# TGoldC/Motion-Planning-for-Autonomous-Driving-with-MPC

Hardware: AMD Instinct MI355X
Metric: MPC steps/sec (N=30, nx=6 nu=2) at batch=4096 (higher is better)
Workload: dtype f64; 1 GPU; N=30 nx=6 nu=2 bicycle lane-following, batch=4096/GPU, tol 1e-8; mode=converged, gpu=AMD Radeon Graphics

## Files before the change

motion-planning-for-autonomous-driving-with-mpc_amd/csrc/mpc_solve_plan.h:

```cpp
#pragma once
#include <algorithm>
#include <cctype>
#include <cstdlib>
#include <cstring>
#include <string>

#include "mpc_host_common.h"

namespace mpc {

struct Knobs {
    int pipeline, hybrid, hybrid_bx, hybrid_live, pipe_help, pipe_test_abort, pipe_xcd_mask, pipe_early;
    int rescue, rescue_wg, rescue_alone, loop_async, sync_spin, max_batch, friction_lb, bound_mask, big_wg, groups, poison;
    int timing;
    Knobs();
};
enum class KnobParse {
    ON,
    INT,
    FLAG,
    MASK,
    FRIC,
};
struct KnobDef { const char* name; int Knobs::*field; int dflt; KnobParse parse; };
inline constexpr KnobDef KNOBS[] = {
    {"pipeline", &Knobs::pipeline, 1, KnobParse::ON},           {"hybrid", &Knobs::hybrid, 1, KnobParse::INT},
    {"hybrid_bx", &Knobs::hybrid_bx, 0, KnobParse::INT},        {"hybrid_live", &Knobs::hybrid_live, -1, KnobParse::INT},
    {"pipe_help", &Knobs::pipe_help, -1, KnobParse::INT},       {"pipe_test_abort", &Knobs::pipe_test_abort, 0, KnobParse::FLAG},
    {"pipe_xcd_mask", &Knobs::pipe_xcd_mask, 0, KnobParse::MASK}, {"rescue", &Knobs::rescue, 1, KnobParse::ON},
    {"rescue_wg", &Knobs::rescue_wg, 1, KnobParse::INT},        {"rescue_alone", &Knobs::rescue_alone, 0, KnobParse::FLAG},
    {"loop_async", &Knobs::loop_async, 1, KnobParse::ON},       {"sync_spin", &Knobs::sync_spin, 1, KnobParse::ON},
    {"max_batch", &Knobs::max_batch, 0, KnobParse::INT},        {"friction_lb", &Knobs::friction_lb, 0, KnobParse::FRIC},
    {"bound_mask", &Knobs::bound_mask, 1, KnobParse::INT},      {"big_wg", &Knobs::big_wg, 0, KnobParse::FLAG},
    {"groups", &Knobs::groups, 0, KnobParse::INT},              {"poison", &Knobs::poison, 0, KnobParse::FLAG},
    {"timing", &Knobs::timing, 0, KnobParse::INT},               {"pipe_early", &Knobs::pipe_early, -1, KnobParse::INT},
};
inline Knobs::Knobs() { for (const KnobDef& e : KNOBS) this->*e.field = e.dflt; }
inline const KnobDef* find_knob(const char* name) {
    for (const KnobDef& e : KNOBS) if (name && strcmp(name, e.name) == 0) return &e;
    return nullptr;
}
inline int set_knob(Knobs& k, const char* name, const char* value) {
    const KnobDef* e = find_knob(name);
    if (!e) return MPC_ERR_INVALID;
    int v = e->dflt;
    if (value) {
        const long iv = strtol(value, nullptr, 0);
        switch (e->parse) {
            case KnobParse::ON: v = value[0] != '0'; break;
            case KnobParse::INT: v = (int)iv; break;
            case KnobParse::FLAG: v = (value[0] == '\0' ? 1 : (int)iv) != 0; break;
            case KnobParse::MASK: v = (int)(uint32_t)strtoul(value, nullptr, 0); break;
            case KnobParse::FRIC: v = strcmp(value, "ipopt") == 0 ? 1 : strcmp(value, "nlp") == 0 ? 0 : (int)iv; break;
        }
    }
    k.*e->field = v;
    return MPC_OK;
}
inline int get_knob(const Knobs& k, const char* name, long* out) {
    const KnobDef* e = find_knob(name);
    if (!e) return MPC_ERR_INVALID;
    *out = e->parse == KnobParse::MASK ? (long)(uint32_t)(k.*e->field) : (long)(k.*e->field);
    return MPC_OK;
}
inline void knobs_from_env(Knobs& k) {
    for (const KnobDef& e : KNOBS) {
        std::string env = "MPCGPU_";
        for (const char* c = e.name; *c; ++c) env += (char)toupper(*c);
        const char* v = getenv(env.c_str());
        if (v) (void)set_knob(k, e.name, v);
    }
}

constexpr int TIMING_STAGE = 1,
              TIMING_PIPE = 2,
              TIMING_WG = 4,
              TIMING_START = 8,
              TIMING_WG_TRACE = 16;

constexpr int STAGE_MAX_THREADS = 512;
constexpr int MAX_GROUPS = 4;
constexpr int MAX_POLL_IT = 1024;
constexpr size_t LDS_MAX = 160 * 1024 - 1024;

#ifndef MPC_STAGE_STASH
#define MPC_STAGE_STASH 1
#endif
template <int NX> struct Stash {
    static constexpr int rows(bool has_ou) { return 4 * (NX + 2) + 2 * 3 + (has_ou ? 2 * 3 : 0) + 3 + 2 * NX; }
};

constexpr uint32_t REF_BOUND_VM = 0x33u;
constexpr uint32_t REF_DENSE_LO = 0x31u, REF_DENSE_HI = 0x33u;

constexpr int RIC_DEPTH = 4;
constexpr int RIC_DEPTH_F = 10;

constexpr uint32_t PIPE_X_STRIDE = 64;
enum PipeXcdWord : uint32_t { PX_ARRIVE = 0, PX_HEAD = 16, PX_TAIL = 32, PX_FINISHED = 48, PX_HO_TICKET = 56 };
constexpr uint32_t PIPE_ABORT = 8 * PIPE_X_STRIDE;
constexpr uint32_t HO_BUCKETS = 4;
enum PipeHeadWord : uint32_t {
    PH_ABORT = 0, PH_ROUNDS = 1,
    PH_STAT64 = 2,
    PH_STAGE_WORKERS = 12, PH_RIC_WORKERS = 13, PH_FAIL = 14,
    PH_WG = 16,
    PH_HELPED = 21, PH_FIN_TICKET = 22,
    PH_HO = 24,
    PH_DETAIL = 28,
    PH_WORDS = 32 };
enum PipeStat64 : uint32_t { P64_RIC_WAIT, P64_STAGE_WAIT, P64_STAGE_BUSY, P64_ITEMS };
enum WgStatWord : uint32_t { WGS_ROUNDS_MAX, WGS_ROUNDS, WGS_SWEEPS, WGS_INST_ROUNDS, WGS_RESCUED, WGS_WORDS };
constexpr uint32_t PIPE_STATS = PIPE_ABORT + PH_STAT64, PIPE_WG = PIPE_ABORT + PH_WG, PIPE_HO = PIPE_ABORT + PH_HO, PIPE_HDR = PIPE_ABORT + PH_WORDS;
struct CtlField { uint32_t at, words, align; };
template <size_t N> constexpr bool ctl_fields_ok(const CtlField (&f)[N], uint32_t size) {
    for (size_t i = 0; i < N; ++i) {
        if (f[i].at % f[i].align || f[i].at + f[i].words > size) return false;
        for (size_t j = 0; j < i; ++j) if (f[i].at < f[j].at + f[j].words && f[j].at < f[i].at + f[i].words) return false;
    }
    return true;
}
constexpr CtlField PIPE_HEAD_FIELDS[] = {{PH_ABORT, 1, 1}, {PH_ROUNDS, 1, 1}, {PH_STAT64, 8, 2}, {PH_STAGE_WORKERS, 1, 1}, {PH_RIC_WORKERS, 1, 1}, {PH_FAIL, 1, 1},
                                         {PH_WG, WGS_WORDS, 1}, {PH_HELPED, 1, 1}, {PH_FIN_TICKET, 1, 1}, {PH_HO, HO_BUCKETS, 1}, {PH_DETAIL, 4, 1}};
constexpr CtlField PIPE_XCD_FIELDS[] = {{PX_ARRIVE, 1, 1}, {PX_HEAD, 1, 1}, {PX_TAIL, 1, 1}, {PX_FINISHED, 1, 1}, {PX_HO_TICKET, 1, 1}};
static_assert(ctl_fields_ok(PIPE_HEAD_FIELDS, PH_WORDS) && PIPE_ABORT % 2 == 0 && PH_HO + HO_BUCKETS <= PH_DETAIL, "the head's fields are disjoint, inside it, the uint64 ones 8-byte aligned; the hand-over counters end in front of the abort details");
static_assert(ctl_fields_ok(PIPE_XCD_FIELDS, PIPE_X_STRIDE), "the fields of an XCD record are disjoint and inside it");
constexpr uint32_t pipe_slots_off(uint32_t ntiles) { return (PIPE_HDR + ntiles + 1u) & ~1u; }
constexpr size_t pipe_step_off(uint32_t ntiles, uint32_t cap) { return (size_t)pipe_slots_off(ntiles) + (size_t)16 * cap; }
constexpr size_t pipe_ctl_words(uint32_t ntiles, uint32_t cap) { return pipe_step_off(ntiles, cap) + (size_t)((ntiles + 1u) & ~1u); }
constexpr uint32_t pipe_item(uint32_t tile, uint32_t q, uint32_t round) { return ((round & 0xFFFFu) << 16) | (tile << 8) | q; }
constexpr uint32_t pipe_item_tile(uint32_t item) { return (item >> 8) & 0xFFu; }
constexpr uint32_t pipe_item_q(uint32_t item) { return item & 0xFFu; }
constexpr uint32_t pipe_item_round(uint32_t item) { return item >> 16; }
constexpr int PIPE_MAX_TILES = 256;
static_assert(PIPE_MAX_TILES <= 256, "a slot's payload has eight bits for the tile");
constexpr int PIPE_LEAD = 18;

constexpr size_t prestart_doubles(int NX, int S, int bx) { return (size_t)4 * S * (NX + 2) + (size_t)(3 * NX + 2) * S * bx + (size_t)4 * bx; }
template <int NX>
struct WgLds {
    static constexpr int PAD = Rec<NX>::SIZE > 64 ? Rec<NX>::SIZE : 64;
    static constexpr size_t doubles(int S, int bxw) { return (size_t)PAD + (size_t)Rec<NX>::SIZE * S * bxw + (size_t)2 * S * (NX + 2) + (size_t)16 * bxw + (size_t)64 * NX + (size_t)WgScl::SIZE * bxw; }
};

struct PlanState {
    int n_cu = 256;
    uint32_t xcd_mask = 0xFFu;
    bool ws_mailbox = false;
    bool pipe_disabled = false;
    bool resc_hint = false;
    int32_t B = 0;
    int32_t per_inst_obst = OBST_SHARED;
    bool trace = false;
    bool in_rescue = false;
    bool async_loop = false;
};
struct SolvePlan {
    bool small_wg;
    int S, bx, threads, nblk, ntiles, G, stash_rows;
    size_t lds_bytes, lds_init, ric_lds;
    bool masked;
    int cap, chunk;
    bool polled;
    bool fused;
    size_t lds_pre, lds_start;
    bool res_path, pipe_path;
    int hyb_bx;
    bool resc_alone, hyb_ok;
    int hand;
    bool wg_resc;
    size_t wg_lds;
    int wg_grid;
    uint32_t xcd_mask;
    int n_xcd, tiles_x, cu_x, n_ric;
    uint32_t pipe_cap;
    bool pipe_help;
    int pipe_lead;
    int mbw_live;
    bool stage_timing, start_timing, wg_timing, wg_trace, pipe_timing, poison;
    size_t max_rows;
    bool mailbox;
    bool rescue;
    bool loop_async;
};

template <int NX>
SolvePlan plan_solve_nx(const HostProblem& hp, const Knobs& kn, const PlanState& st) {
    const mpc_problem_desc& d = hp.desc;
    const int B = st.B;
    SolvePlan pl{};
    const size_t Bp = ((size_t)B + 63) / 64 * 64;
    const int S = d.N + 1;
    pl.S = S;
    pl.ntiles = (int)(Bp / 64);
    const int ntiles = pl.ntiles;
    pl.small_wg = 4 * S <= 256 && !kn.big_wg;
    pl.bx = pick_bx(d.N, pl.small_wg ? 256 : STAGE_MAX_THREADS);
    const int bx = pl.bx;
    pl.threads = ((S * bx + 63) / 64) * 64;
    pl.nblk = (B + bx - 1) / bx;
    pl.stage_timing = (kn.timing & TIMING_STAGE) != 0;
    const int nw = pl.threads / 64;
    pl.stash_rows = pl.small_wg && MPC_STAGE_STASH ? std::max(Stash<NX>::rows(hp.has_ou != 0), 2 * NX) : 2 * NX;
    pl.lds_bytes = ((size_t)nw * 10 * bx + (size_t)2 * S * (NX + 2) + (size_t)pl.stash_rows * pl.threads) * sizeof(double);
    pl.lds_init = ((size_t)nw * 10 * bx + (size_t)2 * S * (NX + 2) + (size_t)2 * NX * pl.threads) * sizeof(double);
    pl.ric_lds = std::max(RIC_DEPTH * (size_t)((MPC_EV(Dim<NX>::NBLK) * 512 + 1023) / 1024) * 1024,
                          RIC_DEPTH_F * (size_t)((Dim<NX>::NKK * 512 + 1023) / 1024 + 6) * 1024) + 64;
    pl.G = 1;
    if (!st.trace && !pl.stage_timing && kn.groups > 0) pl.G = std::min(std::max(std::min(kn.groups, ntiles / 4), 1), MAX_GROUPS);
    const int G = pl.G;
    const bool ref_vm_ok = ((hp.lo_mask | hp.hi_mask) & ~REF_BOUND_VM) == 0u;
    pl.masked = kn.bound_mask != 0 && ref_vm_ok && (hp.dense_mask & REF_DENSE_LO) == REF_DENSE_LO && ((hp.dense_mask >> 8) & REF_DENSE_HI) == REF_DENSE_HI &&
                hp.has_ol && !hp.has_ou && d.obst_mult == 3 && st.per_inst_obst == OBST_SHARED;
    pl.cap = d.fixed_iters > 0 ? d.fixed_iters : d.max_iter;
    pl.chunk = d.fixed_iters > 0 ? pl.cap : 4;
    pl.polled = d.fixed_iters <= 0 && !st.trace;
    const int n_w = 2 * d.N + NX * (d.N + 1);
    pl.lds_pre = prestart_doubles(NX, S, bx) * sizeof(double);
    const size_t lds_in = (size_t)bx * (2 * n_w - 2 * d.N) * sizeof(double);
    const size_t lds_red = (size_t)(pl.threads / 64) * 10 * bx * sizeof(double);
    pl.fused = lds_red + pl.lds_pre + 16 + lds_in <= 78 * 1024 && d.N >= 1 && pl.small_wg;
    pl.lds_start = std::max(lds_red + pl.lds_pre + 16 + lds_in, pl.lds_init);

    auto wg_lds = [&](int bxw) {
        const size_t pre = prestart_doubles(NX, S, bxw) * sizeof(double);
        const size_t init = ((size_t)10 * bxw + (size_t)2 * S * (NX + 2) + (size_t)2 * NX * 64) * sizeof(double);
        return std::max(WgLds<NX>::doubles(S, bxw) * sizeof(double), bxw == 1 ? std::max(pre, init) : (size_t)0);
    };
    pl.rescue = kn.rescue && d.fixed_iters <= 0 && !st.trace && hp.has_ol && hp.ol_raw > 0.0;
    const bool resc_cond = pl.rescue && (kn.rescue_wg >= 2 || kn.rescue_alone || (kn.rescue_wg == 1 && st.resc_hint)) && !st.in_rescue;
    int hyb_bx = ((kn.hybrid_bx == 2 || (kn.hybrid_bx == 0 && B > 4 * st.n_cu)) && S * 2 <= 64) ? 2 : 1;
    if (kn.hybrid_bx == 0 && resc_cond && hyb_bx == 2 && (size_t)ntiles * 64 * 8 <= (size_t)4 * st.n_cu * 18) hyb_bx = 1;
    pl.resc_alone = kn.rescue_alone && kn.hybrid_bx == 0 && kn.hybrid_live < 0 && resc_cond && ntiles <= 128;
    if (pl.resc_alone || st.in_rescue) hyb_bx = 1;
    pl.hyb_bx = hyb_bx;
    pl.wg_resc = resc_cond && hyb_bx == 1;
    pl.wg_lds = wg_lds(hyb_bx);
    pl.mailbox = pl.small_wg && S <= 64 && kn.hybrid && d.fixed_iters <= 0 && kn.pipeline && !st.pipe_disabled;
    pl.hyb_ok = kn.hybrid && st.ws_mailbox && d.fixed_iters <= 0 && kn.pipeline && !st.pipe_disabled && G == 1 && pl.small_wg && S <= 64 &&
                pl.wg_lds <= LDS_MAX / 4 && !st.trace && !pl.stage_timing;
    int hand = 0;
    if (pl.hyb_ok) {
        const int base = std::min(64, 4 * st.n_cu * hyb_bx / std::max(1, ntiles));
        hand = base >= 64 ? base : std::max(base, std::min(50, base < 32 ? 7 * base / 4 : 3 * base / 2));
        if (hyb_bx == 1 && base < 64 && hand < 40) hand = 40;
        if ((size_t)ntiles * 64 * 8 <= (size_t)4 * st.n_cu * hyb_bx * (hyb_bx == 2 ? 9 : 18)) hand = 64;
        if (pl.resc_alone) hand = 64;
        if (kn.hybrid_live >= 0) hand = std::min(64, kn.hybrid_live);
    }
// ... 91 lines not shown
```

motion-planning-for-autonomous-driving-with-mpc_amd/csrc/mpcgpu.hip:

```cpp
#include <hip/hip_runtime.h>
#include <type_traits>

#include <algorithm>
#include <cctype>
#include <cstdio>
#include <cstdlib>
#include <cstring>
#include <new>
#include <string>
#include <vector>

#include "mpc_host_common.h"
#include "mpc_solve_plan.h"
#include "mpc_stamps.h"
#include "mpc_closed_loop.h"
#include "mpc_forces_qp.h"
#include "mpc_riccati_mfma.h"
#include "mpc_sens.h"
#include "mpc_loop_lin.h"

using namespace mpc;

namespace {

// ... 156 lines not shown
        if (!bounds_in_lds) lds_barrier();
        if (!__any(c.active ? 1 : 0)) return;
        MPC_STAMP(P.DBG, blockIdx.x, SB_LOADED, t == 0 && stamp);
        Red1 r1;
        phase_step_candidates<NX, VM>(P, c, r1);
        MPC_STAMP(P.DBG, blockIdx.x, SB_P1, t == 0 && stamp);
        block_reduce(r1, bx, lds);
        phase_linesearch_begin<NX>(P, c, r1);
        MPC_STAMP(P.DBG, blockIdx.x, SB_RED1, t == 0 && stamp);
        double* stash = lds_x;
        if (STASH) stash_xfer<NX, true, VM>(c, stash, blockDim.x, t, has_ou);
        while (__any((c.active && c.searching) ? 1 : 0)) {
            Red2 r2;
            phase_trial_eval<NX, VM>(P, c, r2);
            block_reduce(r2, bx, lds);
            phase_linesearch_decide<NX>(P, c, r2);
        }
        if (STASH) stash_xfer<NX, false, VM>(c, stash, blockDim.x, t, has_ou);
        MPC_STAMP(P.DBG, blockIdx.x, SB_LS, t == 0 && stamp);
        phase_apply_update<NX, false, VM>(P, c);
        MPC_STAMP(P.DBG, blockIdx.x, SB_UPDATE, t == 0 && stamp);
    }
    {
        double* ex = lds_x;
        const int T = blockDim.x;
#pragma unroll
        for (int i = 0; i < NX; ++i) { ex[i * T + t] = c.z[2 + i]; ex[(NX + i) * T + t] = c.lam[i]; }
        lds_barrier();
        const int tn = t + bx;
        if (tn < T) {
#pragma unroll
            for (int i = 0; i < NX; ++i) { c.xn[i] = ex[i * T + tn]; c.lamn[i] = ex[(NX + i) * T + tn]; }
        }
    }
    MPC_STAMP(P.DBG, blockIdx.x, SB_XCHG, t == 0 && stamp);
    Red3 r3;
    phase_eval_assemble<NX, !INIT, false, VM>(P, c, r3);
    MPC_STAMP(P.DBG, blockIdx.x, SB_EVAL, t == 0 && stamp);
    block_reduce(r3, bx, lds);
    MPC_STAMP(P.DBG, blockIdx.x, SB_RED3, t == 0 && stamp);
    phase_finish<NX, false>(P, c, r3, n_mult, n_z);
    MPC_STAMP(P.DBG, blockIdx.x, SB_END, t == 0 && stamp);
    if (live_out != nullptr && t < 64) {
        const unsigned long long m = __ballot((c.valid && c.k == 0 && c.active && c.status == ST_RUNNING) ? 1 : 0);
        if (t == 0) *live_out = (uint32_t)m;
    }
    if (P.run_counter != nullptr && t < 64) {
        const int cnt = __popcll(__ballot((c.valid && c.k == 0 && c.active && c.status == ST_RUNNING) ? 1 : 0));
        if (t == 0 && cnt) atomicAdd(P.run_counter, cnt);
    }
}

struct WgIo { uint32_t fail; uint32_t ill; double* c0; double* rn; double* r0; double* scl; bool fric, have; };
template <int NX, uint32_t VM, class Mid>
__device__ __forceinline__ void wg_stage(const PRef& P, const int ib0, const int ib1, double* lds_bnd, const mpc_lds_ptr rec_base, const int n_mult, const int n_z, const bool stamp,
                                         uint32_t* live_out, WgIo& io, Mid&& mid) {
    const int bx = P.bx, t = threadIdx.x;
    Ctx<NX> c;
    PreTmp<NX> tmp;
    c.k = t / bx;
    c.bl = t & (bx - 1);
    c.mb = (int)blockIdx.x * bx;
    c.b = c.bl ? ib1 : ib0;
    c.valid = (c.k <= P.N) && (c.b >= 0) && (c.b < P.B);
    c.active = false;
    c.ill = false;
    c.status = 0;
    c.iters = 0;
    c.rec = rec_base + ((t & (bx - 1)) * (P.N + 1) + (c.k <= P.N ? c.k : 0)) * Rec<NX>::SIZE;
    c.bnd = (mpc_lds_cptr)(lds_ptr_t)lds_bnd;
    c.bnd_ub = (P.N + 1) * (NX + 2);
    c.scl = (mpc_lds_ptr)(lds_ptr_t)(io.scl + c.bl * WgScl::SIZE);
    mid();
    phase_load_scalars<NX, true>(P, c);
    if (io.have) {
        phase_preload<NX, true, VM, false, true>(P, c, tmp, io.fric);
#pragma unroll
        for (int i = 0; i < NX; ++i) { c.rn[i] = io.rn[t * NX + i]; c.r0[i] = c.k == 0 ? io.r0[c.bl * 8 + i] : 0.0; }
    } else {
        phase_preload<NX, true, VM, false>(P, c, tmp);
#pragma unroll
        for (int i = 0; i < NX; ++i) { io.rn[t * NX + i] = c.rn[i]; if (c.k == 0 && c.valid) io.r0[c.bl * 8 + i] = c.r0[i]; }
        io.fric = __ballot((c.valid && c.k == 0 && c.fric_row) ? 1 : 0) != 0ull;
    }
    MPC_STAMP(P.DBG, blockIdx.x, SB_ENTER, t == 0 && stamp);
    if (((io.fail >> (t & (bx - 1))) & 1u) && c.valid) { c.status = -7; c.active = false; }
    phase_preload_rec<NX>(P, c, tmp);
    phase_premath<NX>(P, c, tmp);
    MPC_STAMP(P.DBG, blockIdx.x, SB_ISSUED, t == 0 && stamp);
    if (!__any(c.active ? 1 : 0)) return;
    MPC_STAMP(P.DBG, blockIdx.x, SB_LOADED, t == 0 && stamp);
    Red1 r1;
    phase_step_candidates<NX, VM>(P, c, r1);
    MPC_STAMP(P.DBG, blockIdx.x, SB_P1, t == 0 && stamp);
    block_reduce(r1, bx, nullptr);
    phase_linesearch_begin<NX>(P, c, r1);
    MPC_STAMP(P.DBG, blockIdx.x, SB_RED1, t == 0 && stamp);
    while (__any((c.active && c.searching) ? 1 : 0)) {
        Red2 r2;
        phase_trial_eval<NX, VM>(P, c, r2);
        block_reduce(r2, bx, nullptr);
        phase_linesearch_decide<NX, true>(P, c, r2);
    }
    MPC_STAMP(P.DBG, blockIdx.x, SB_LS, t == 0 && stamp);
    phase_apply_update<NX, true, VM>(P, c);
    MPC_STAMP(P.DBG, blockIdx.x, SB_UPDATE, t == 0 && stamp);
    {
        const int tn = t + bx;
#pragma unroll
        for (int i = 0; i < NX; ++i) {
            const double xs = __shfl_down(c.z[2 + i], (unsigned)bx, 64), ls = __shfl_down(c.lam[i], (unsigned)bx, 64);
            if (tn < 64) { c.xn[i] = xs; c.lamn[i] = ls; }
        }
    }
    MPC_STAMP(P.DBG, blockIdx.x, SB_XCHG, t == 0 && stamp);
    Red3 r3;
    phase_eval_assemble<NX, true, true, VM>(P, c, r3);
    {
        const unsigned long long bal = __ballot((c.active && c.ill) ? 1 : 0);
        const unsigned long long col0 = ~0ull / ((1ull << bx) - 1ull);
        if (c.active && (bal & (col0 << (t & (bx - 1)))) != 0ull && t < bx) MPC_S(P.ISC, IS_ILL) = 1;
        io.ill |= ((bal & col0) != 0ull ? 1u : 0u) | ((bx > 1 && (bal & (col0 << 1)) != 0ull) ? 2u : 0u);
        if (c.k == 0 && c.active) {
#pragma unroll
            for (int i = 0; i < NX; ++i) io.c0[(t & (bx - 1)) * 8 + i] = c.z[2 + i] - c.r0[i];
        }
    }
    MPC_STAMP(P.DBG, blockIdx.x, SB_EVAL, t == 0 && stamp);
    block_reduce(r3, bx, nullptr);
    MPC_STAMP(P.DBG, blockIdx.x, SB_RED3, t == 0 && stamp);
    phase_finish<NX, true>(P, c, r3, n_mult, n_z);
    MPC_STAMP(P.DBG, blockIdx.x, SB_END, t == 0 && stamp);
    {
        const unsigned long long m = __ballot((c.valid && c.k == 0 && c.active && c.status == ST_RUNNING) ? 1 : 0);
        if (t == 0) *live_out = (uint32_t)m;
    }
}

template <int NX, bool INIT, int MAXT, uint32_t VM = 0xFFu>
__global__ void __launch_bounds__(MAXT, (INIT && MAXT <= 256) ? 2 : 1) k_stage(const Params Pk, const int n_mult, const int n_z, const int stash_rows) {
    const PRef P(Pk);
    extern __shared__ __attribute__((aligned(16))) double lds[];
    uint32_t blk = blockIdx.x;
    if ((gridDim.x & 7u) == 0u) blk = (blk & 7u) * (gridDim.x >> 3) + (blk >> 3);
    const uint32_t b0 = (blk + (uint32_t)P.tile0 * (64u / (uint32_t)P.bx)) * (uint32_t)P.bx;
    const unsigned long long bits = (!INIT && P.tile_mask != nullptr) ? P.tile_mask[b0 >> 6] : ~0ull;
    stage_block<NX, INIT, MAXT, VM>(P, n_mult, n_z, stash_rows, b0, bits, lds);
}

constexpr int32_t HO_IN_MB = 0x40000000;

template <int NCH>
__device__ __forceinline__ void wait_dma_behind(int stages_behind) {
    if (stages_behind >= 4 && 4 * NCH <= 63) asm volatile("s_waitcnt vmcnt(%0)" ::"n"(4 * NCH <= 63 ? 4 * NCH : 0) : "memory");
    else if (stages_behind >= 3 && 3 * NCH <= 63) asm volatile("s_waitcnt vmcnt(%0)" ::"n"(3 * NCH <= 63 ? 3 * NCH : 0) : "memory");
    else if (stages_behind >= 2) asm volatile("s_waitcnt vmcnt(%0)" ::"n"(2 * NCH) : "memory");
    else if (stages_behind == 1) asm volatile("s_waitcnt vmcnt(%0)" ::"n"(NCH) : "memory");
    else asm volatile("s_waitcnt vmcnt(0)" ::: "memory");
}

__device__ __forceinline__ void ho_lists(const PRef& P, const uint32_t bb, int32_t* ho_list, uint32_t* ho_count, const uint32_t* tile_word) {
#if defined(__HIP_DEVICE_COMPILE__)
    const int lane = threadIdx.x & 63;
    const bool active = (int)bb < P.B && (int32_t)MPC_U(P.ISC, (uint32_t)IS_STATUS) == ST_RUNNING;
    if (__ballot(active ? 1 : 0) == 0ull) return;
    const int32_t in_mb = (tile_word != nullptr && (__hip_atomic_load(tile_word + (bb >> 6), __ATOMIC_RELAXED, __HIP_MEMORY_SCOPE_AGENT) >> 31)) ? HO_IN_MB : 0;
    const double e0 = active ? (double)MPC_U(P.SC, (uint32_t)SC_E0) : 0.0;
    const int bucket = e0 >= 1e-3 ? 0 : e0 >= 1e-4 ? 1 : e0 >= 1e-5 ? 2 : 3;
    for (int q = 0; q < (int)HO_BUCKETS; ++q) {
        const unsigned long long mq = __ballot((active && bucket == q) ? 1 : 0);
        if (mq == 0ull) continue;
        uint32_t base = 0u;
        if (lane == 0) base = __hip_atomic_fetch_add(ho_count + q, (uint32_t)__popcll(mq), __ATOMIC_RELAXED, __HIP_MEMORY_SCOPE_AGENT);
        base = (uint32_t)__builtin_amdgcn_readfirstlane((int)base);
        if (active && bucket == q) ho_list[(uint32_t)q * (uint32_t)P.Bp + base + (uint32_t)__popcll(mq & ((1ull << lane) - 1ull))] = (int32_t)bb | in_mb;
    }
#endif
}

struct RicNoPublish {
    __device__ __forceinline__ uint32_t last_pass(unsigned long long) const { return 0u; }
    __device__ __forceinline__ void publish(uint32_t) const {}
};
template <int NX, class Pub = RicNoPublish>
__device__ __forceinline__ unsigned long long riccati_tile(const PRef& P, const uint32_t tile, char* smem, const bool stamp = true, const int handover_live = 0,
                                                           const int kpub = -1, const Pub& pub = Pub()) {
#if defined(__HIP_DEVICE_COMPILE__)
    using D = Dim<NX>;
    constexpr int NS = D::NS;
    constexpr uint32_t BLK_BYTES = MPC_EV(D::NBLK) * 512u;
    constexpr int BLK_CHUNKS = (BLK_BYTES + 1023u) / 1024u;
    constexpr uint32_t SLOT = BLK_CHUNKS * 1024u;
    constexpr int KK_CHUNKS = (D::NKK * 512u + 1023u) / 1024u;
    constexpr int FWD_CHUNKS = KK_CHUNKS + 6;
    constexpr uint32_t FSLOT = FWD_CHUNKS * 1024u;
    static_assert(2 * BLK_CHUNKS <= 63 && RIC_DEPTH == 4 && 4 * FWD_CHUNKS <= 63 && RIC_DEPTH_F == 10, "vmcnt is a 6-bit counter");
    constexpr uint32_t RING_BYTES = (RIC_DEPTH * SLOT > RIC_DEPTH_F * FSLOT) ? RIC_DEPTH * SLOT : RIC_DEPTH_F * FSLOT;
    int* flag = reinterpret_cast<int*>(smem + RING_BYTES);
    const int wave = __builtin_amdgcn_readfirstlane((int)(threadIdx.x >> 6));
    const int lane = threadIdx.x & 63;
    const int b = (int)(tile * 64u) + lane;
    const uint32_t bb = (uint32_t)b;
    const int N = P.N;
    const bool active = (b < P.B) && ((int32_t)MPC_U(P.ISC, (uint32_t)IS_STATUS) == ST_RUNNING);
    const unsigned long long act_mask = __ballot(active ? 1 : 0);
    if (act_mask == 0ull) return 0ull;
    if (__popcll(act_mask) * 64 < handover_live * min(64, P.B - (int)(tile * 64u)) + 64) return 0ull;
    MPC_STAMP(P.DBG, blockIdx.x, RT_BEGIN, threadIdx.x == 0 && stamp);
    const __amdgpu_buffer_rsrc_t rsrc = P.rws;
    const uint32_t tile_off = tile * P.tile_elems * 8u;
    const uint32_t blk_base = (uint32_t)(uintptr_t)P.BLK - (uint32_t)(uintptr_t)P.WS + tile_off;
    const uint32_t kk_base = (uint32_t)(uintptr_t)P.KK - (uint32_t)(uintptr_t)P.WS + tile_off;
    auto dma = [&](uint32_t src_, uint32_t dst_, int nchunks) {
        const uint32_t src = (uint32_t)__builtin_amdgcn_readfirstlane((int)src_), dst = (uint32_t)__builtin_amdgcn_readfirstlane((int)dst_);
#pragma unroll
        for (int c = 0; c < nchunks; ++c)
        {
            if (P.xcu) __builtin_amdgcn_raw_ptr_buffer_load_lds(rsrc, (lds_ptr_t)(smem + dst + (uint32_t)c * 1024u), 16, lane * 16, (int)(src + (uint32_t)c * 1024u), 0, MPC_AUX_SC1);
            else __builtin_amdgcn_raw_ptr_buffer_load_lds(rsrc, (lds_ptr_t)(smem + dst + (uint32_t)c * 1024u), 16, lane * 16, (int)(src + (uint32_t)c * 1024u), 0, 0);
        }
    };
    auto lds_r = [&](uint32_t off, uint32_t r) { return *reinterpret_cast<const double*>(smem + off + mpc_prow(r) * 8u + (uint32_t)lane * 16u); };
    auto read_stage = [&](uint32_t slot, RicStage<NX>& s) {
#pragma unroll
        for (int i = 0; i < NX; ++i) {
#pragma unroll
            for (int j = i; j < NX; ++j)
                s.H[D::sidx(i, j)] = (D::hrow(i, j) >= 0) ? lds_r(slot, D::B_H + (D::hrow(i, j) >= 0 ? D::hrow(i, j) : 0)) : 0.0;
        }
        s.ruu[0] = lds_r(slot, D::B_RUU);
        s.ruu[1] = lds_r(slot, D::B_RUU + 1);
#pragma unroll
        for (int i = 0; i < 6; ++i) s.a[i] = lds_r(slot, D::B_A + i);
#pragma unroll
        for (int i = 0; i < NX; ++i) { s.gx[i] = lds_r(slot, D::B_GX + i); s.cn[i] = lds_r(slot, D::B_CN + i); }
        s.gu[0] = lds_r(slot, D::B_GU);
        s.gu[1] = lds_r(slot, D::B_GU + 1);
    };
    double delta = 0.0, delta_last = 0.0, hux0 = 0.0, hux1 = 0.0;
    bool need = false, failed = false;
    if (wave == 0 || wave == 2) {
        need = active;
        if (active) { delta_last = MPC_U(P.SC, (uint32_t)SC_DLAST); hux0 = MPC_U(P.SC, (uint32_t)SC_HUX0); hux1 = MPC_U(P.SC, (uint32_t)SC_HUX1); }
    }
    for (;;) {
        if (wave >= 3) {
            for (int t = 0; t <= N; ++t) lds_barrier();
        } else if (wave == 1) {
            for (int j = 0; j < RIC_DEPTH - 1 && j <= N; ++j) dma(blk_base + (uint32_t)(N - j) * BLK_BYTES, (uint32_t)j * SLOT, BLK_CHUNKS);
            for (int t = 0; t <= N; ++t) {
                const int k = N - t;
                wait_dma_behind<BLK_CHUNKS>(k < RIC_DEPTH - 2 ? k : RIC_DEPTH - 2);
                lds_barrier();
                const int kn = k - (RIC_DEPTH - 1);
                if (kn >= 0) dma(blk_base + (uint32_t)kn * BLK_BYTES, (uint32_t)((t + RIC_DEPTH - 1) % RIC_DEPTH) * SLOT, BLK_CHUNKS);
            }
        } else {
            bool ok = need;
            const bool sym = delta != 0.0 || delta_last != 0.0;
            auto sweep = [&](auto sym_tag, auto ne_tag, auto vec_tag) {
                constexpr bool SYM = decltype(sym_tag)::value;
                constexpr int NE = decltype(ne_tag)::value;
                constexpr bool VEC = decltype(vec_tag)::value;
                const bool lead = !VEC && threadIdx.x == 0 && stamp;
                double Ps[NS], pv[NX];
                for (int t = 0; t <= N; ++t) {
                    const int k = N - t;
                    if (t == 15) MPC_STAMP(P.DBG, blockIdx.x, RT_B15_WAIT, lead);
                    lds_barrier();
                    if (t == 15) MPC_STAMP(P.DBG, blockIdx.x, RT_B15_GO, lead);
                    RicStage<NX> s;
                    read_stage((uint32_t)(t % RIC_DEPTH) * SLOT, s);
                    if (t == 0) {
#pragma unroll
                        for (int i = 0; i < NS; ++i) Ps[i] = s.H[i];
#pragma unroll
                        for (int i = 0; i < NX; ++i) { Ps[D::sidx(i, i)] += delta; pv[i] = s.gx[i]; }
                        if (ok) {
                            if (VEC) ric_store_vector_pk<NX>(P, bb, N, Ps, pv);
                            else ric_store_matrix_pk<NX>(P, bb, N, Ps);
                        }
                    } else if (ok) {
                        RicGain<NX> g;
                        if (VEC) {
                            double Pn[NS];
#pragma unroll
                            for (int i = 0; i < NS; ++i) Pn[i] = Ps[i];
                            ok = ric_matrix_step<NX, NE, SYM>(P, k, s, delta, hux0, hux1, Ps, g, SYM && sym);
                            if (ok) {
                                ric_vector_step<NX, NE, SYM>(P, s, Pn, g, pv);
                                ric_store_vector<NX>(P, bb, k, Ps, pv, g);
                            }
                        } else {
                            ok = ric_matrix_step<NX, NE, SYM>(P, k, s, delta, hux0, hux1, Ps, g, SYM && sym);
                            if (ok) ric_store_matrix<NX>(P, bb, k, Ps, g);
                        }
                    }
                    if (t == 15) MPC_STAMP(P.DBG, blockIdx.x, RT_B15_END, lead);
                }
            };
            auto sweep_as = [&](auto vec_tag) {
                if (__any(sym ? 1 : 0)) sweep(std::true_type{}, std::integral_constant<int, NX>{}, vec_tag);
                else if (NX == 6 && P.dec_s) sweep(std::false_type{}, std::integral_constant<int, (NX == 6 ? 5 : NX)>{}, vec_tag);
                else sweep(std::false_type{}, std::integral_constant<int, NX>{}, vec_tag);
            };
            if (wave == 0) sweep_as(std::false_type{});
            else sweep_as(std::true_type{});
            if (need && ok) need = false;
            else if (need) {
                if (delta == 0.0) delta = (delta_last == 0.0) ? DW_0 : fmax(DW_MIN, KW_MINUS * delta_last);
                else delta *= (delta_last == 0.0) ? KW_PLUS_BAR : KW_PLUS;
                if (delta > DW_MAX) { need = false; failed = true; }
            }
            int again = 0;
            uint32_t pub_word = 0u;
            if (wave == 0) {
                again = __any(need ? 1 : 0);
                if (!again) {
                    if (active && failed) MPC_U(P.ISC, (uint32_t)IS_STATUS) = P.emit ? ST_SWEEP_FAILED : -7;
                    if (active && !failed) {
                        if (delta > 0.0) MPC_U(P.SC, (uint32_t)SC_DLAST) = delta;
                        MPC_U(P.SC, (uint32_t)SC_DELTA) = delta;
                    }
                    pub_word = pub.last_pass(act_mask);
                }
            }
            asm volatile("s_waitcnt vmcnt(0)" ::: "memory");
            if (wave == 0 && lane == 0) { flag[0] = again; flag[1] = (int)pub_word; }
        }
        lds_barrier();
        const int again = lds_uniform(*flag);
        lds_barrier();
        if (!again) break;
    }
    MPC_STAMP(P.DBG, blockIdx.x, RT_BWD_END, threadIdx.x == 0 && stamp);
    const bool go = (wave == 0) && active && !failed;
    if (wave >= 3) {
        for (int k = 0; k < N; ++k) lds_barrier();
    } else if (wave >= 1) {
        const int par = wave - 1;
        auto dma_fwd = [&](int k, uint32_t dst) {
            dma(kk_base + (uint32_t)k * (D::NKK * 512u), dst, KK_CHUNKS);
            static_assert(D::B_A % 2 == 0 && D::B_CN % 2 == 0 && D::NKK % 2 == 0, "sub-blocks copied on their own start on a row-pair boundary");
            dma(blk_base + (uint32_t)k * BLK_BYTES + D::B_A * 512u, dst + KK_CHUNKS * 1024u, 3);
            dma(blk_base + (uint32_t)k * BLK_BYTES + D::B_CN * 512u, dst + (KK_CHUNKS + 3) * 1024u, 3);
        };
        for (int j = par; j < RIC_DEPTH_F - 1 && j < N; j += 2) dma_fwd(j, (uint32_t)j * FSLOT);
        for (int k = 0; k < N; ++k) {
            if ((k & 1) == par) {
                const int last = (N - 1 < k + RIC_DEPTH_F - 2) ? N - 1 : k + RIC_DEPTH_F - 2;
                wait_dma_behind<FWD_CHUNKS>((last - k) >> 1);
            }
            lds_barrier();
            if (k == kpub && wave == 1) pub.publish((uint32_t)flag[1]);
            const int kn = k + RIC_DEPTH_F - 1;
            if (kn < N && (kn & 1) == par) dma_fwd(kn, (uint32_t)(kn % RIC_DEPTH_F) * FSLOT);
        }
    } else {
        double dx[NX];
#pragma unroll
        for (int i = 0; i < NX; ++i) dx[i] = go ? -(double)MPC_U(P.SC, (uint32_t)(SC_C0 + i)) : 0.0;
        for (int k = 0; k < N; ++k) {
            const uint32_t slot = (uint32_t)(k % RIC_DEPTH_F) * FSLOT;
            if (k == 15) MPC_STAMP(P.DBG, blockIdx.x, RT_F15_WAIT, threadIdx.x == 0 && stamp);
            lds_barrier();
            if (k == 15) MPC_STAMP(P.DBG, blockIdx.x, RT_F15_GO, threadIdx.x == 0 && stamp);
            if (k == 0) MPC_STAMP(P.DBG, blockIdx.x, RT_F0, threadIdx.x == 0 && stamp);
            FwdStage<NX> f;
#pragma unroll
            for (int j = 0; j < NX; ++j) {
                f.K0[j] = lds_r(slot, (uint32_t)j);
                f.K1[j] = lds_r(slot, (uint32_t)(NX + j));
                f.cn[j] = lds_r(slot + (KK_CHUNKS + 3) * 1024u, (uint32_t)j);
            }
            f.kf0 = lds_r(slot, (uint32_t)(2 * NX));
            f.kf1 = lds_r(slot, (uint32_t)(2 * NX + 1));
#pragma unroll
            for (int i = 0; i < 6; ++i) f.a[i] = lds_r(slot + KK_CHUNKS * 1024u, (uint32_t)i);
            riccati_forward_step<NX>(P, bb, k, f, dx);
            if (k == 15) MPC_STAMP(P.DBG, blockIdx.x, RT_F15_END, threadIdx.x == 0 && stamp);
        }
        if (go) {
            double dz[D::NZ];
            dz[0] = 0.0;
            dz[1] = 0.0;
#pragma unroll
            for (int i = 0; i < NX; ++i) dz[2 + i] = dx[i];
            ws_store_rows<D::NZ>(MPC_ROWS(MPC_UK(P.DZ, D::NZ, N, e)), dz);
        }
    }
    MPC_STAMP(P.DBG, blockIdx.x, RT_FWD_END, threadIdx.x == 0 && stamp);
    return act_mask;
#else
    return 0ull;
#endif
}

template <int NX>
__global__ void __launch_bounds__(192) k_riccati(const Params Pk) {
    const PRef P(Pk);
    extern __shared__ __attribute__((aligned(16))) char smem[];
    const uint32_t tile = blockIdx.x + (uint32_t)P.tile0;
    const unsigned long long act_mask = riccati_tile<NX>(P, tile, smem);
    if (P.tile_mask != nullptr && threadIdx.x == 0) P.tile_mask[tile] = act_mask;
}

struct PipeArgs {
    uint32_t* ctl;
    uint32_t ntiles;
    uint32_t xcd_mask;
    uint32_t n_ric;
    uint32_t cap;
    uint32_t items;
    uint32_t handover;
    int32_t* ho_list;
    uint32_t flags;
    uint32_t lead;
};
constexpr uint32_t PIPE_EXIT = 0xFFFFFFFFu;
constexpr unsigned long long PIPE_SPIN_LIMIT = 5000000ull;
#ifndef MPC_PIPE_SLEEP
#define MPC_PIPE_SLEEP 8
#endif

__device__ __forceinline__ void pipe_acquire() {
#if defined(__HIP_DEVICE_COMPILE__)
    __builtin_amdgcn_fence(__ATOMIC_ACQUIRE, "workgroup");
#endif
}
__device__ __forceinline__ uint32_t pipe_ld(const uint32_t* p) { return __hip_atomic_load(p, __ATOMIC_RELAXED, __HIP_MEMORY_SCOPE_AGENT); }
__device__ __forceinline__ void pipe_st(uint32_t* p, uint32_t v) { __hip_atomic_store(p, v, __ATOMIC_RELAXED, __HIP_MEMORY_SCOPE_AGENT); }
__device__ __forceinline__ uint32_t pipe_add(uint32_t* p, uint32_t v) { return __hip_atomic_fetch_add(p, v, __ATOMIC_RELAXED, __HIP_MEMORY_SCOPE_AGENT); }

struct PipeStepWait {
    const uint32_t* word;
    uint32_t* abort_w;
    uint32_t* sh;
    uint32_t want, tile;
    bool late;
    __device__ __forceinline__ bool there() const { return late; }
    __device__ __forceinline__ bool operator()() const {
#if defined(__HIP_DEVICE_COMPILE__)
        if (threadIdx.x == 0) {
            uint32_t ok = 1u;
            const unsigned long long t0 = wall_clock64();
            for (;;) {
                const uint32_t seen = pipe_ld(word);
                if (((seen - want) & 0xFFFFu) < 0x8000u) break;
                if (pipe_ld(abort_w)) { ok = 0u; break; }
                if (wall_clock64() - t0 > PIPE_SPIN_LIMIT) { pipe_st(abort_w + PH_DETAIL, (tile << 16) | want); pipe_st(abort_w + PH_DETAIL + 1, seen); pipe_st(abort_w + PH_DETAIL + 3, (uint32_t)(wall_clock64() - t0)); pipe_st(abort_w, 5u); ok = 0u; break; }
                __builtin_amdgcn_s_sleep(MPC_PIPE_SLEEP);
            }
            pipe_acquire();
            *sh = ok;
        }
        lds_barrier();
        return lds_uniform(*sh) != 0u;
#else
        return true;
#endif
    }
};
struct PipePublish {
    unsigned long long* tile_mask_w;
    uint32_t* tail;
    unsigned long long* slots;
    uint32_t items, cap, tile, round;
    bool early;
    __device__ __forceinline__ uint32_t last_pass(unsigned long long mask) const {
        uint32_t tk = 0u;
        if ((threadIdx.x & 63) == 0) {
            __hip_atomic_store(tile_mask_w, mask, __ATOMIC_RELAXED, __HIP_MEMORY_SCOPE_AGENT);
            if (early) tk = pipe_add(tail, items);
        }
        return tk;
    }
    __device__ __forceinline__ void publish(uint32_t tk) const {
        const uint32_t q = threadIdx.x & 63u;
        if (q < items) __hip_atomic_store(slots + ((tk + q) & (cap - 1u)), ((unsigned long long)(tk + q + 1u) << 32) | (unsigned long long)pipe_item(tile, q, round + 1u), __ATOMIC_RELAXED, __HIP_MEMORY_SCOPE_AGENT);
    }
};

__global__ void __launch_bounds__(256) k_copy16(const uint4* __restrict__ src, uint4* __restrict__ dst, size_t n) {
    const size_t stride = (size_t)gridDim.x * 1024;
    size_t i = (size_t)blockIdx.x * 1024 + threadIdx.x;
    for (; i + 768 < n; i += stride) {
        const uint4 a = src[i], b = src[i + 256], c = src[i + 512], d = src[i + 768];
        dst[i] = a; dst[i + 256] = b; dst[i + 512] = c; dst[i + 768] = d;
    }
    for (; i < n; i += 256) dst[i] = src[i];
}

__global__ void k_poison(double* ws, uint32_t tile_elems, uint32_t ntiles, uint32_t e0, uint32_t e1) {
    const size_t n = (size_t)(e1 - e0) * ntiles;
    for (size_t i = (size_t)blockIdx.x * blockDim.x + threadIdx.x; i < n; i += (size_t)gridDim.x * blockDim.x) {
        const size_t tile = i / (e1 - e0), e = e0 + i % (e1 - e0);
        ws[tile * tile_elems + e] = __builtin_nan("");
    }
}

__global__ void k_xcd_census(uint32_t* mask) {
#if defined(__HIP_DEVICE_COMPILE__)
    if (threadIdx.x == 0) atomicOr(mask, 1u << ((uint32_t)__builtin_amdgcn_s_getreg((3 << 11) | 20) & 15u));
#endif
}

template <int NX, int VAR, bool HELP = false>
__global__ void __launch_bounds__(256) k_pipeline(const Params Pk, const PipeArgs A, const int n_mult, const int n_z, const int stash_rows) {
    const PRef P = mpc_pref(Pk, true);
#if defined(__HIP_DEVICE_COMPILE__)
    extern __shared__ __attribute__((aligned(16))) double lds[];
    __shared__ uint32_t sh_word[4];
    const int t = threadIdx.x;
    const uint32_t xcc = (uint32_t)__builtin_amdgcn_s_getreg((3 << 11) | 20) & 15u;
    if (!((A.xcd_mask >> xcc) & 1u)) return;
    const uint32_t n_xcd = (uint32_t)__popc(A.xcd_mask), xcd = (uint32_t)__popc(A.xcd_mask & ((1u << xcc) - 1u));
    uint32_t* X = A.ctl + xcd * PIPE_X_STRIDE;
    uint32_t* abort_w = A.ctl + PIPE_ABORT;
    uint32_t* stage_done = A.ctl + PIPE_HDR;
    unsigned long long* slots = reinterpret_cast<unsigned long long*>(A.ctl + pipe_slots_off(A.ntiles)) + (size_t)xcd * A.cap;
    uint32_t* step_ready = A.ctl + pipe_step_off(A.ntiles, A.cap);
    const int kpub = (!HELP && A.lead > 0u && P.N > 0) ? max(P.N - (int)A.lead, 0) : -1;
    const uint32_t n_tiles_x = A.ntiles > xcd ? (A.ntiles - xcd + n_xcd - 1u) / n_xcd : 0u;
    if (n_tiles_x == 0u) return;
    if ((A.flags & 2u) && t == 0) pipe_st(abort_w, 1u);
    if (t == 0) sh_word[0] = pipe_add(X + PX_ARRIVE, 1u);
    lds_barrier();
    const uint32_t slot = lds_uniform(sh_word[0]);
    const uint32_t n_ric = A.n_ric < n_tiles_x ? A.n_ric : n_tiles_x;
    lds_barrier();
    unsigned long long waited = 0;
    uint32_t n_pass = 0;
    if (slot < n_ric) {
// ... 3774 lines not shown
```

Baseline: 5.762 million MPC steps/s.

## Group forward Riccati stages in pairs and prefill early forward slots during backward pass

The forward sweep now processes two stages per LDS barrier, prefetching the next stage's gains from LDS while computing the current one, which halves the barrier count. The first RIC_PRO stages' gain rows are written to LDS directly by the compute wave during the backward pass, and their A/cn sub-blocks are DMA'd by the backward loader, so the forward sweep can start without waiting for a fresh prologue. The initial state C0 is also read during the last backward pass instead of after it. This adds a more intricate ring-slot schedule and vmcnt accounting, and it requires the forward ring to avoid overlapping the backward ring.

```diff
diff --git a/motion-planning-for-autonomous-driving-with-mpc_amd/csrc/mpc_ric_ring.h b/motion-planning-for-autonomous-driving-with-mpc_amd/csrc/mpc_ric_ring.h
--- /dev/null
+++ b/motion-planning-for-autonomous-driving-with-mpc_amd/csrc/mpc_ric_ring.h
@@ -0,0 +1,40 @@
+#pragma once
+
+namespace mpc {
+
+constexpr int RIC_DEPTH = 4;
+constexpr int RIC_DEPTH_F = 10;
+constexpr int RIC_PRO = 4;
+constexpr int RIC_GROUP = 2;
+
+constexpr int ric_imin(int a, int b) { return a < b ? a : b; }
+constexpr int ric_imax(int a, int b) { return a > b ? a : b; }
+
+constexpr int ric_wait_stages(int nch, int behind) { return behind >= 4 && 4 * nch <= 63 ? 4 : behind >= 3 && 3 * nch <= 63 ? 3 : behind >= 2 ? 2 : behind == 1 ? 1 : 0; }
+
+constexpr int ric_bwd_barriers(int N) { return N + 1; }
+constexpr int ric_bwd_slot(int t) { return t % RIC_DEPTH; }
+constexpr int ric_bwd_first(int N) { return ric_imin(RIC_DEPTH - 1, N + 1); }
+constexpr int ric_bwd_behind(int N, int t) { return ric_imin(N - t, RIC_DEPTH - 2); }
+constexpr int ric_bwd_request(int N, int t) { return t + RIC_DEPTH - 1 <= N ? t + RIC_DEPTH - 1 : -1; }
+constexpr int ric_pro_len(int N) { return ric_imin(N, RIC_PRO); }
+constexpr int ric_pro_static(int N, int t) { return t < ric_pro_len(N) ? t : -1; }
+
+constexpr int ric_fwd_slot(int k) { return (k + RIC_DEPTH_F - RIC_PRO) % RIC_DEPTH_F; }
+constexpr int ric_fwd_groups(int N) { return (N + RIC_GROUP - 1) / RIC_GROUP; }
+constexpr int ric_fwd_landed(int N, int g) { return ric_imin(N - 1, RIC_GROUP * g + 2); }
+constexpr int ric_fwd_done(int g) { return RIC_GROUP * g - 1; }
+constexpr int ric_fwd_requested(int N, int g) { return ric_imin(N - 1, ric_imax(RIC_DEPTH_F - 1, g >= 1 ? ric_fwd_done(g - 1) + RIC_DEPTH_F : 0)); }
+constexpr int ric_fwd_behind(int N, int g, int par) {
+    int n = 0;
+    for (int k = ric_imax(ric_fwd_landed(N, g) + 1, RIC_PRO); k <= ric_fwd_requested(N, g); ++k) n += (k & 1) == par;
+    return n;
+}
+constexpr int ric_fwd_pub_group(int kpub) { return kpub / RIC_GROUP; }
+
+constexpr bool ric_ring_fits(unsigned bwd_slot, unsigned fwd_slot) { return (unsigned)(RIC_DEPTH_F - RIC_PRO) * fwd_slot >= (unsigned)RIC_DEPTH * bwd_slot; }
+
+static_assert(RIC_GROUP == 2 && RIC_PRO % RIC_GROUP == 0 && RIC_PRO >= RIC_GROUP + 1 && RIC_PRO < RIC_DEPTH_F,
+              "two loaders of alternate stages; what the compute wave reads behind barrier 0 (stages 0 .. 2) is prologue");
+
+}
diff --git a/motion-planning-for-autonomous-driving-with-mpc_amd/csrc/mpc_solve_plan.h b/motion-planning-for-autonomous-driving-with-mpc_amd/csrc/mpc_solve_plan.h
--- a/motion-planning-for-autonomous-driving-with-mpc_amd/csrc/mpc_solve_plan.h
+++ b/motion-planning-for-autonomous-driving-with-mpc_amd/csrc/mpc_solve_plan.h
@@ -6,6 +6,7 @@
 #include <string>
 
 #include "mpc_host_common.h"
+#include "mpc_ric_ring.h"
 
 namespace mpc {
 
@@ -93,8 +94,6 @@
 constexpr uint32_t REF_BOUND_VM = 0x33u;
 constexpr uint32_t REF_DENSE_LO = 0x31u, REF_DENSE_HI = 0x33u;
 
-constexpr int RIC_DEPTH = 4;
-constexpr int RIC_DEPTH_F = 10;
 
 constexpr uint32_t PIPE_X_STRIDE = 64;
 enum PipeXcdWord : uint32_t { PX_ARRIVE = 0, PX_HEAD = 16, PX_TAIL = 32, PX_FINISHED = 48, PX_HO_TICKET = 56 };
diff --git a/motion-planning-for-autonomous-driving-with-mpc_amd/csrc/mpcgpu.hip b/motion-planning-for-autonomous-driving-with-mpc_amd/csrc/mpcgpu.hip
--- a/motion-planning-for-autonomous-driving-with-mpc_amd/csrc/mpcgpu.hip
+++ b/motion-planning-for-autonomous-driving-with-mpc_amd/csrc/mpcgpu.hip
@@ -332,10 +332,11 @@
 
 template <int NCH>
 __device__ __forceinline__ void wait_dma_behind(int stages_behind) {
-    if (stages_behind >= 4 && 4 * NCH <= 63) asm volatile("s_waitcnt vmcnt(%0)" ::"n"(4 * NCH <= 63 ? 4 * NCH : 0) : "memory");
-    else if (stages_behind >= 3 && 3 * NCH <= 63) asm volatile("s_waitcnt vmcnt(%0)" ::"n"(3 * NCH <= 63 ? 3 * NCH : 0) : "memory");
-    else if (stages_behind >= 2) asm volatile("s_waitcnt vmcnt(%0)" ::"n"(2 * NCH) : "memory");
-    else if (stages_behind == 1) asm volatile("s_waitcnt vmcnt(%0)" ::"n"(NCH) : "memory");
+    const int w = ric_wait_stages(NCH, stages_behind);
+    if (w == 4) asm volatile("s_waitcnt vmcnt(%0)" ::"n"(4 * NCH <= 63 ? 4 * NCH : 0) : "memory");
+    else if (w == 3) asm volatile("s_waitcnt vmcnt(%0)" ::"n"(3 * NCH <= 63 ? 3 * NCH : 0) : "memory");
+    else if (w == 2) asm volatile("s_waitcnt vmcnt(%0)" ::"n"(2 * NCH) : "memory");
+    else if (w == 1) asm volatile("s_waitcnt vmcnt(%0)" ::"n"(NCH) : "memory");
     else asm volatile("s_waitcnt vmcnt(0)" ::: "memory");
 }
 
@@ -374,7 +375,8 @@
     constexpr int KK_CHUNKS = (D::NKK * 512u + 1023u) / 1024u;
     constexpr int FWD_CHUNKS = KK_CHUNKS + 6;
     constexpr uint32_t FSLOT = FWD_CHUNKS * 1024u;
-    static_assert(2 * BLK_CHUNKS <= 63 && RIC_DEPTH == 4 && 4 * FWD_CHUNKS <= 63 && RIC_DEPTH_F == 10, "vmcnt is a 6-bit counter");
+    static_assert(3 * BLK_CHUNKS + 6 <= 63 && RIC_DEPTH == 4 && 4 * FWD_CHUNKS <= 63 && RIC_DEPTH_F == 10, "vmcnt is a 6-bit counter");
+    static_assert(ric_ring_fits(SLOT, FSLOT), "the prologue's forward slots are written while the backward ring is in use");
     constexpr uint32_t RING_BYTES = (RIC_DEPTH * SLOT > RIC_DEPTH_F * FSLOT) ? RIC_DEPTH * SLOT : RIC_DEPTH_F * FSLOT;
     int* flag = reinterpret_cast<int*>(smem + RING_BYTES);
     const int wave = __builtin_amdgcn_readfirstlane((int)(threadIdx.x >> 6));
@@ -400,7 +402,20 @@
             else __builtin_amdgcn_raw_ptr_buffer_load_lds(rsrc, (lds_ptr_t)(smem + dst + (uint32_t)c * 1024u), 16, lane * 16, (int)(src + (uint32_t)c * 1024u), 0, 0);
         }
     };
-    auto lds_r = [&](uint32_t off, uint32_t r) { return *reinterpret_cast<const double*>(smem + off + mpc_prow(r) * 8u + (uint32_t)lane * 16u); };
+    auto dma_fwd_static = [&](int k) {
+        static_assert(D::B_A % 2 == 0 && D::B_CN % 2 == 0 && D::NKK % 2 == 0, "sub-blocks copied on their own start on a row-pair boundary");
+        const uint32_t dst = (uint32_t)ric_fwd_slot(k) * FSLOT;
+        dma(blk_base + (uint32_t)k * BLK_BYTES + D::B_A * 512u, dst + KK_CHUNKS * 1024u, 3);
+        dma(blk_base + (uint32_t)k * BLK_BYTES + D::B_CN * 512u, dst + (KK_CHUNKS + 3) * 1024u, 3);
+    };
+    auto dma_fwd = [&](int k) {
+        dma(kk_base + (uint32_t)k * (D::NKK * 512u), (uint32_t)ric_fwd_slot(k) * FSLOT, KK_CHUNKS);
+        dma_fwd_static(k);
+    };
+    auto pro_write = [&](int k, int pair, double r0, double r1) {
+        *reinterpret_cast<double2*>(smem + (uint32_t)ric_fwd_slot(k) * FSLOT + (uint32_t)pair * 1024u + (uint32_t)lane * 16u) = make_double2(r0, r1);
+    };
+    auto lds_r =[&](uint32_t off, uint32_t r) { return *reinterpret_cast<const double*>(smem + off + mpc_prow(r) * 8u + (uint32_t)lane * 16u); };
     auto read_stage = [&](uint32_t slot, RicStage<NX>& s) {
 #pragma unroll
         for (int i = 0; i < NX; ++i) {
@@ -419,21 +434,25 @@
     };
     double delta = 0.0, delta_last = 0.0, hux0 = 0.0, hux1 = 0.0;
     bool need = false, failed = false;
+    double c0v[NX];
     if (wave == 0 || wave == 2) {
         need = active;
         if (active) { delta_last = MPC_U(P.SC, (uint32_t)SC_DLAST); hux0 = MPC_U(P.SC, (uint32_t)SC_HUX0); hux1 = MPC_U(P.SC, (uint32_t)SC_HUX1); }
     }
     for (;;) {
+#pragma unroll
+        for (int i = 0; i < NX; ++i) c0v[i] = 0.0;
         if (wave >= 3) {
-            for (int t = 0; t <= N; ++t) lds_barrier();
+            for (int t = 0; t < ric_bwd_barriers(N); ++t) lds_barrier();
         } else if (wave == 1) {
-            for (int j = 0; j < RIC_DEPTH - 1 && j <= N; ++j) dma(blk_base + (uint32_t)(N - j) * BLK_BYTES, (uint32_t)j * SLOT, BLK_CHUNKS);
-            for (int t = 0; t <= N; ++t) {
-                const int k = N - t;
-                wait_dma_behind<BLK_CHUNKS>(k < RIC_DEPTH - 2 ? k : RIC_DEPTH - 2);
+            for (int j = 0; j < ric_bwd_first(N); ++j) dma(blk_base + (uint32_t)(N - j) * BLK_BYTES, (uint32_t)ric_bwd_slot(j) * SLOT, BLK_CHUNKS);
+            for (int t = 0; t < ric_bwd_barriers(N); ++t) {
+                wait_dma_behind<BLK_CHUNKS>(ric_bwd_behind(N, t));
                 lds_barrier();
-                const int kn = k - (RIC_DEPTH - 1);
-                if (kn >= 0) dma(blk_base + (uint32_t)kn * BLK_BYTES, (uint32_t)((t + RIC_DEPTH - 1) % RIC_DEPTH) * SLOT, BLK_CHUNKS);
+                const int tn = ric_bwd_request(N, t);
+                if (tn >= 0) dma(blk_base + (uint32_t)(N - tn) * BLK_BYTES, (uint32_t)ric_bwd_slot(tn) * SLOT, BLK_CHUNKS);
+                const int kp = ric_pro_static(N, t);
+                if (kp >= 0) dma_fwd_static(kp);
             }
         } else {
             bool ok = need;
@@ -470,10 +489,17 @@
                             if (ok) {
                                 ric_vector_step<NX, NE, SYM>(P, s, Pn, g, pv);
                                 ric_store_vector<NX>(P, bb, k, Ps, pv, g);
+                                if (k < RIC_PRO) pro_write(k, NX, g.kf0, g.kf1);
                             }
                         } else {
                             ok = ric_matrix_step<NX, NE, SYM>(P, k, s, delta, hux0, hux1, Ps, g, SYM && sym);
-                            if (ok) ric_store_matrix<NX>(P, bb, k, Ps, g);
+                            if (ok) {
+                                ric_store_matrix<NX>(P, bb, k, Ps, g);
+                                if (k < RIC_PRO) {
+#pragma unroll
+                                    for (int q = 0; q < NX; ++q) pro_write(k, q, 2 * q < NX ? g.K0[2 * q] : g.K1[2 * q - NX], 2 * q + 1 < NX ? g.K0[2 * q + 1] : g.K1[2 * q + 1 - NX]);
+                                }
+                            }
                         }
                     }
                     if (t == 15) MPC_STAMP(P.DBG, blockIdx.x, RT_B15_END, lead);
@@ -503,9 +529,15 @@
                         MPC_U(P.SC, (uint32_t)SC_DELTA) = delta;
                     }
                     pub_word = pub.last_pass(act_mask);
+                    if (active && !failed) {
+#pragma unroll
+                        for (int i = 0; i < NX; ++i) c0v[i] = (double)MPC_U(P.SC, (uint32_t)(SC_C0 + i));
+                    }
                 }
             }
             asm volatile("s_waitcnt vmcnt(0)" ::: "memory");
+#pragma unroll
+            for (int i = 0; i < NX; ++i) asm volatile("" : "+v"(c0v[i]));
             if (wave == 0 && lane == 0) { flag[0] = again; flag[1] = (int)pub_word; }
         }
         lds_barrier();
@@ -515,38 +547,26 @@
     }
     MPC_STAMP(P.DBG, blockIdx.x, RT_BWD_END, threadIdx.x == 0 && stamp);
     const bool go = (wave == 0) && active && !failed;
+    const int G = ric_fwd_groups(N);
     if (wave >= 3) {
-        for (int k = 0; k < N; ++k) lds_barrier();
+        for (int g = 0; g < G; ++g) lds_barrier();
     } else if (wave >= 1) {
         const int par = wave - 1;
-        auto dma_fwd = [&](int k, uint32_t dst) {
-            dma(kk_base + (uint32_t)k * (D::NKK * 512u), dst, KK_CHUNKS);
-            static_assert(D::B_A % 2 == 0 && D::B_CN % 2 == 0 && D::NKK % 2 == 0, "sub-blocks copied on their own start on a row-pair boundary");
-            dma(blk_base + (uint32_t)k * BLK_BYTES + D::B_A * 512u, dst + KK_CHUNKS * 1024u, 3);
-            dma(blk_base + (uint32_t)k * BLK_BYTES + D::B_CN * 512u, dst + (KK_CHUNKS + 3) * 1024u, 3);
-        };
-        for (int j = par; j < RIC_DEPTH_F - 1 && j < N; j += 2) dma_fwd(j, (uint32_t)j * FSLOT);
-        for (int k = 0; k < N; ++k) {
-            if ((k & 1) == par) {
-                const int last = (N - 1 < k + RIC_DEPTH_F - 2) ? N - 1 : k + RIC_DEPTH_F - 2;
-                wait_dma_behind<FWD_CHUNKS>((last - k) >> 1);
-            }
+        for (int j = RIC_PRO + par; j <= ric_fwd_requested(N, 0); j += 2) dma_fwd(j);
+        const int gpub = kpub >= 0 ? ric_fwd_pub_group(kpub) : -1;
+        for (int g = 0; g < G; ++g) {
+            wait_dma_behind<FWD_CHUNKS>(ric_fwd_behind(N, g, par));
             lds_barrier();
-            if (k == kpub && wave == 1) pub.publish((uint32_t)flag[1]);
-            const int kn = k + RIC_DEPTH_F - 1;
-            if (kn < N && (kn & 1) == par) dma_fwd(kn, (uint32_t)(kn % RIC_DEPTH_F) * FSLOT);
+            if (g == gpub && wave == 1) pub.publish((uint32_t)flag[1]);
+            for (int kn = ric_fwd_requested(N, g) + 1; kn <= ric_fwd_requested(N, g + 1); ++kn)
+                if ((kn & 1) == par) dma_fwd(kn);
         }
     } else {
         double dx[NX];
 #pragma unroll
-        for (int i = 0; i < NX; ++i) dx[i] = go ? -(double)MPC_U(P.SC, (uint32_t)(SC_C0 + i)) : 0.0;
-        for (int k = 0; k < N; ++k) {
-            const uint32_t slot = (uint32_t)(k % RIC_DEPTH_F) * FSLOT;
-            if (k == 15) MPC_STAMP(P.DBG, blockIdx.x, RT_F15_WAIT, threadIdx.x == 0 && stamp);
-            lds_barrier();
-            if (k == 15) MPC_STAMP(P.DBG, blockIdx.x, RT_F15_GO, threadIdx.x == 0 && stamp);
-            if (k == 0) MPC_STAMP(P.DBG, blockIdx.x, RT_F0, threadIdx.x == 0 && stamp);
-            FwdStage<NX> f;
+        for (int i = 0; i < NX; ++i) dx[i] = go ? -c0v[i] : 0.0;
+        auto read_fwd = [&](int k, FwdStage<NX>& f) {
+            const uint32_t slot = (uint32_t)ric_fwd_slot(k) * FSLOT;
 #pragma unroll
             for (int j = 0; j < NX; ++j) {
                 f.K0[j] = lds_r(slot, (uint32_t)j);
@@ -557,8 +577,24 @@
             f.kf1 = lds_r(slot, (uint32_t)(2 * NX + 1));
 #pragma unroll
             for (int i = 0; i < 6; ++i) f.a[i] = lds_r(slot + KK_CHUNKS * 1024u, (uint32_t)i);
-            riccati_forward_step<NX>(P, bb, k, f, dx);
-            if (k == 15) MPC_STAMP(P.DBG, blockIdx.x, RT_F15_END, threadIdx.x == 0 && stamp);
+        };
+        FwdStage<NX> fa, fb;
+        for (int k = 0; k < N; k += RIC_GROUP) {
+            const bool st15 = k == 14 && N > 15 && threadIdx.x == 0 && stamp;
+            MPC_STAMP(P.DBG, blockIdx.x, RT_F15_WAIT, st15);
+            lds_barrier();
+            MPC_STAMP(P.DBG, blockIdx.x, RT_F15_GO, st15);
+            if (k == 0) {
+                MPC_STAMP(P.DBG, blockIdx.x, RT_F0, threadIdx.x == 0 && stamp);
+                read_fwd(0, fa);
+            }
+            if (k + 1 < N) read_fwd(k + 1, fb);
+            riccati_forward_step<NX>(P, bb, k, fa, dx);
+            if (k + 2 < N) read_fwd(k + 2, fa);
+#pragma unroll
+            for (int i = 0; i < NX; ++i) asm volatile("" : "+v"(dx[i]));
+            if (k + 1 < N) riccati_forward_step<NX>(P, bb, k + 1, fb, dx);
+            MPC_STAMP(P.DBG, blockIdx.x, RT_F15_END, st15);
         }
         if (go) {
             double dz[D::NZ];
```

Measured after the change: 5.777 million MPC steps/s, median of 3. Within noise of the previous version (+0.3%).
